# vsois/hanabi-agents

Measured on AMD Instinct MI355X. Metric: env_steps_per_sec, higher is better.
Workload: dtype u8 env/encoder + bfloat16 Q-net GEMM (fp32 accumulate, fp32 master weights)

## Files before the change

### hanabi-agents_amd/csrc/learner2.hip

```cpp
#include <hip/hip_runtime.h>
#include <hip/hip_bf16.h>
#include <hip/hip_fp16.h>

#include <cstdint>
#include <type_traits>

#include "../../include/hanabi_hip.h"
#include "adam_rule.hpp"
#include "common.hpp"

using hb::fail;

namespace {

template <typename T> __device__ __forceinline__ float ld(const T* p, long long i);
template <> __device__ __forceinline__ float ld<float>(const float* p, long long i) { return p[i]; }
template <> __device__ __forceinline__ float ld<__hip_bfloat16>(const __hip_bfloat16* p, long long i) { return __bfloat162float(p[i]); }
template <> __device__ __forceinline__ float ld<__half>(const __half* p, long long i) { return __half2float(p[i]); }
template <typename T> __device__ __forceinline__ void st(T* p, long long i, float v);
template <> __device__ __forceinline__ void st<float>(float* p, long long i, float v) { p[i] = v; }
template <> __device__ __forceinline__ void st<__hip_bfloat16>(__hip_bfloat16* p, long long i, float v) { p[i] = __float2bfloat16(v); }
template <> __device__ __forceinline__ void st<__half>(__half* p, long long i, float v) { p[i] = __float2half(v); }

template <typename T> __device__ __forceinline__ float rounded(float v);
// ... 503 lines not shown
  else return __bfloat162float(b[i]);
}
template <bool F16>
__device__ __forceinline__ tg_f32x4 tg_mfma(const uint4& wv, const uint4& xv, const tg_f32x4& c) {
  if constexpr (F16) {
    union { uint4 u; tg_f16x8 f; } w, x;
    w.u = wv; x.u = xv;
    return __builtin_amdgcn_mfma_f32_16x16x32_f16(w.f, x.f, c, 0, 0, 0);
  } else {
    union { uint4 u; tg_bf16x8 f; } w, x;
    w.u = wv; x.u = xv;
    return __builtin_amdgcn_mfma_f32_16x16x32_bf16(w.f, x.f, c, 0, 0, 0);
  }
}
template <bool F16>
__global__ __launch_bounds__(64) void thin_gemm_kernel(const ThinArgs a, const int batch) {
  const int lane = threadIdx.x;
  const unsigned lr = lane & 15, kq = lane >> 4;
  const unsigned ct = blockIdx.y + a.n_tiles;
  const unsigned c = ct * 16u + 4u * kq;
  const unsigned half = 32u * a.ldx;
#pragma unroll 1
  for (int z = 0; z < batch; ++z) {
    float b0 = 0.f, b1 = 0.f, b2 = 0.f, b3 = 0.f;
    if (a.bias) {
      const __hip_bfloat16* bz = a.bias + static_cast<size_t>(z) * a.nb;
      b0 = tg_bias<F16>(bz, c); b1 = tg_bias<F16>(bz, c + 1); b2 = tg_bias<F16>(bz, c + 2); b3 = tg_bias<F16>(bz, c + 3);
    }
    const unsigned xo = (z * a.x_bs + (blockIdx.x * 32u + lr) * a.ldx + kq * 8u) * 2u;
    const unsigned wo = (z * a.w_bs + (ct * 16u + lr) * a.ldw + kq * 8u) * 2u;
// ... 21 lines not shown
      *reinterpret_cast<uint2*>(o) = make_uint2(tg_pack<F16>(v[0], v[1]), tg_pack<F16>(v[2], v[3]));
      *reinterpret_cast<uint2*>(o + 16u * static_cast<size_t>(a.ldo)) = make_uint2(tg_pack<F16>(v[4], v[5]), tg_pack<F16>(v[6], v[7]));
    }
  }
}

struct TailArgs {
  hb::adam::AdamMulti adam;
  const unsigned char* x;
  const unsigned char* dh;
  unsigned char* dw1;
  int batch, k_rows, hidden;
  unsigned ldx, dh_ld, dw1_ld;
  int g_adam;
  int col_tiles;
};
constexpr int kTailLd = 264;

__device__ __forceinline__ void tail_scatter(uint16_t* lds, int col, int b, const uint4& v) {
  const uint32_t w[4] = {v.x, v.y, v.z, v.w};
#pragma unroll
  for (int i = 0; i < 4; ++i) {
    lds[(col + 2 * i) * kTailLd + b] = static_cast<uint16_t>(w[i] & 0xFFFFu);
    lds[(col + 2 * i + 1) * kTailLd + b] = static_cast<uint16_t>(w[i] >> 16);
  }
}

template <bool F16, int W>
__global__ __launch_bounds__(256) void learner_tail_l2_dw1_kernel(const TailArgs a) {
  typedef typename std::conditional<F16, __half, __hip_bfloat16>::type T;
// ... 1 lines not shown
  __shared__ __attribute__((aligned(16))) uint16_t dt[64 * kTailLd];
  const int tid = static_cast<int>(threadIdx.x);
  if (static_cast<int>(blockIdx.x) < a.g_adam) {
    hb::adam::step_block<T, W>(a.adam, static_cast<int>(blockIdx.x), tid);
    return;
  }
  const int tile = static_cast<int>(blockIdx.x) - a.g_adam;
  const int rt = tile / a.col_tiles, ctile = tile - rt * a.col_tiles;
  const int r0 = rt * 32, c0 = ctile * 64;
  const int kb = (a.batch + 31) & ~31;
  uint4 xv[4], dv[8];
#pragma unroll
  for (int it = 0; it < 4; ++it) {
    const int c = tid + it * 256, b = c >> 2, col = r0 + (c & 3) * 8;
    xv[it] = make_uint4(0u, 0u, 0u, 0u);
    if (b < a.batch && col < a.k_rows) xv[it] = *reinterpret_cast<const uint4*>(a.x + (static_cast<size_t>(b) * a.ldx + col) * 2u);
  }
#pragma unroll
  for (int it = 0; it < 8; ++it) {
    const int c = tid + it * 256, b = c >> 3, col = c0 + (c & 7) * 8;
    dv[it] = make_uint4(0u, 0u, 0u, 0u);
    if (b < a.batch && col < a.hidden) dv[it] = *reinterpret_cast<const uint4*>(a.dh + (static_cast<size_t>(b) * a.dh_ld + col) * 2u);
  }
#pragma unroll
  for (int it = 0; it < 4; ++it) {
    const int c = tid + it * 256, b = c >> 2;
    if (b < kb) tail_scatter(xt, (c & 3) * 8, b, xv[it]);
  }
#pragma unroll
  for (int it = 0; it < 8; ++it) {
    const int c = tid + it * 256, b = c >> 3;
// ... 134 lines not shown
      acc0 = tg_mfma<F16>(w0, x0, acc0);
      acc1 = tg_mfma<F16>(w0, x1, acc1);
      acc0 = tg_mfma<F16>(u0, y0, acc0);
      acc1 = tg_mfma<F16>(u0, y1, acc1);
    }
    if (kb < kend) {
      const uint4 x0 = *reinterpret_cast<const uint4*>(a.x + (xo0 + kb)), x1 = *reinterpret_cast<const uint4*>(a.x + (xo1 + kb));
      const uint4 w0 = *reinterpret_cast<const uint4*>(a.wt + (wo0 + kb));
      acc0 = tg_mfma<F16>(w0, x0, acc0);
      acc1 = tg_mfma<F16>(w0, x1, acc1);
    }
    const size_t ob = z * static_cast<size_t>(a.o_bs) + 4u * kq;
    const size_t o0 = ob + static_cast<size_t>(r0) * a.ldo, o1 = ob + static_cast<size_t>(r1) * a.ldo;
    const __hip_bfloat16* bz = a.bias ? a.bias + static_cast<size_t>(z) * a.nb + 4u * kq : nullptr;
    tf_store<F16>(a.out, a.relu, bz, t0 * 16u, o0, o1, v0, v1, acc0, acc1);
  }
}

}

extern "C" {

int hb_c51_loss_sparse(const void* logits_online_dev, const void* logits_target_dev, int32_t dtype, const int32_t* act_dev,
                       const float* rew_dev, const float* term_dev, const double* prios_dev, const float* beta_dev,
                       const float* disc_dev, int32_t mask_terminal, const float* support_dev, int64_t batch, int32_t n_actions,
                       int32_t n_atoms, int32_t row_stride, float* td_dev, float* w_dev, float* dl_dev, float* update_counter_dev,
                       const void* bias_online_dev, const void* bias_target_dev, void* stream) {
  if (!logits_online_dev || !logits_target_dev || !act_dev || !rew_dev || !term_dev || !prios_dev || !beta_dev || !disc_dev ||
      !support_dev || !td_dev || !w_dev || !dl_dev)
    return fail(HB_ERR_INVALID, "null argument");
// ... 45 lines not shown
  }
  HB_HIP(hipGetLastError());
  return HB_OK;
}

int hb_thin_forward(int32_t layer, const void* x_dev, const void* wt_dev, const void* bias_dev, void* out_dev, const int32_t* act_dev,
                    int64_t batch, int32_t n, int32_t k, int32_t ldx, int32_t ldw, int32_t ldo, int64_t x_batch_stride,
                    int64_t w_batch_stride, int64_t out_batch_stride, int32_t n_actions, int32_t n_atoms, int32_t relu, void* stream) {
  if (!x_dev || !wt_dev || !out_dev) return fail(HB_ERR_INVALID, "null argument");
  if (layer != 1 && layer != 2) return fail(HB_ERR_INVALID, "layer must be 1 or 2");
  if (batch <= 0 || n <= 0) return HB_OK;
  const int64_t m = 2 * batch;
  const int nz = layer == 2 ? 2 : 1;
  if (batch % 32 || n % (layer == 1 ? 32 : 16) || k % 32 || k < 32)
    return fail(HB_ERR_INVALID, "need batch % 32 == 0, n % 16 == 0 (layer 1: n % 32 == 0), k % 32 == 0");
  if (ldx < k || ldw < k || ldo < n || ldx % 8 || ldw % 8 || ldo % 4) return fail(HB_ERR_INVALID, "bad leading dimensions");
  if (relu < 0 || relu > 7) return fail(HB_ERR_INVALID, "relu: bit 0 = ReLU, bit 1 = fp32 output, bit 2 = fp16 (not bf16) operands");
  if ((reinterpret_cast<uintptr_t>(x_dev) & 15u) || (reinterpret_cast<uintptr_t>(wt_dev) & 15u) ||
      (reinterpret_cast<uintptr_t>(out_dev) & ((relu & 2) ? 15u : 7u)))
    return fail(HB_ERR_ALIGN, "x / wt must be 16-byte aligned, out 8-byte (fp32 output: 16-byte) aligned");
  if (layer == 2) {
    if (!act_dev) return fail(HB_ERR_INVALID, "null argument");
    if (batch > 256) return fail(HB_ERR_INVALID, "batch must be <= 256 (a wavefront keeps the batch's actions in four registers per lane)");
    if (n_actions < 1 || n_actions > 64 || n_atoms < 1 || n_atoms > 64 || n_actions * n_atoms > n)
      return fail(HB_ERR_INVALID, "need n_actions <= 64, n_atoms <= 64, n_actions * n_atoms <= n");
    if (x_batch_stride < 0 || w_batch_stride < 0 || out_batch_stride < 0) return fail(HB_ERR_INVALID, "negative batch stride");
    if (x_batch_stride % 8 || w_batch_stride % 8 || out_batch_stride % 4) return fail(HB_ERR_INVALID, "batch strides must keep the alignment");
  }
  const int64_t xe = (nz - 1) * x_batch_stride + m * static_cast<int64_t>(ldx), we = (nz - 1) * w_batch_stride + n * static_cast<int64_t>(ldw);
  if (xe >= (1LL << 30) || we >= (1LL << 30)) return fail(HB_ERR_INVALID, "operands beyond the kernel's 32-bit offsets");
  FwdArgs a{};
  a.x = static_cast<const unsigned char*>(x_dev);
  a.wt = static_cast<const unsigned char*>(wt_dev);
  a.bias = static_cast<const __hip_bfloat16*>(bias_dev);
  a.out = out_dev;
// ... 11 lines not shown
    a.reg0_units = a.nrt * (ncp / 2u);
    a.n_units = a.reg0_units + a.nrt * ncp;
  } else {
    a.x_bs = static_cast<unsigned>(x_batch_stride); a.w_bs = static_cast<unsigned>(w_batch_stride); a.o_bs = static_cast<unsigned>(out_batch_stride);
    a.A = n_actions; a.K = n_atoms;
    a.npair = static_cast<unsigned>((n_atoms + 14) / 16 + 1);
    const unsigned groups = a.nrt + static_cast<unsigned>(n_actions < batch ? n_actions : batch);
    a.n_gather = groups * a.npair;
    a.z[0] = 0u; a.z[1] = 1u;
    a.row0[0] = a.row0[1] = static_cast<unsigned>(batch);
    a.reg0_units = a.nrt * ncp;
    a.n_units = a.n_gather + 2u * a.reg0_units;
  }
  const unsigned per = (a.n_units + 1023u) / 1024u;
  a.stride = (a.n_units + per - 1u) / per;
  if (relu & 4) hipLaunchKernelGGL((thin_forward_kernel<true>), dim3(a.stride), dim3(64), 0, static_cast<hipStream_t>(stream), a);
  else hipLaunchKernelGGL((thin_forward_kernel<false>), dim3(a.stride), dim3(64), 0, static_cast<hipStream_t>(stream), a);
  HB_HIP(hipGetLastError());
  return HB_OK;
}

int hb_dqn_loss_sparse(const void* q_online_dev, const void* q_target_dev, int32_t dtype, const int32_t* act_dev, const float* rew_dev,
                       const float* term_dev, const double* prios_dev, const float* beta_dev, const float* disc_dev, int64_t batch,
                       int32_t n_actions, int32_t col_stride, int32_t row_stride, float* td_dev, float* w_dev, float* dl_dev,
                       const void* bias_online_dev, const void* bias_target_dev, void* stream) {
  if (!q_online_dev || !q_target_dev || !act_dev || !rew_dev || !term_dev || !prios_dev || !beta_dev || !disc_dev || !td_dev ||
      !w_dev || !dl_dev)
    return fail(HB_ERR_INVALID, "null argument");
  if (batch <= 0) return HB_OK;
  if (batch > 256) return fail(HB_ERR_INVALID, "batch must be <= 256");
  if (n_actions < 1 || col_stride < 1 || row_stride < (n_actions - 1) * col_stride + 1) return fail(HB_ERR_INVALID, "bad action layout");
// ... 40 lines not shown

}

int hb::adam::launch_tail(const hb_adam_tensor* steps, int n_steps, const hb_adam_tensor& prod, const float* step_dev,
                          float step_offset, int eff_dtype, float lr, float beta1, float beta2, float eps, void* stream) {
  const int dtype = prod.grad_dtype;
  if (!prod.gdh || !prod.grad) return fail(HB_ERR_INVALID, "gradient product: null gdh / grad");
  if (dtype != 1 && dtype != 2) return fail(HB_ERR_INVALID, "gradient product: grad_dtype must be 1 (bf16) or 2 (f16)");
  if (eff_dtype != dtype) return fail(HB_ERR_INVALID, "gradient product: eff_dtype must equal the product's grad_dtype");
  if (prod.g_batch < 1 || prod.g_batch > 256)
    return fail(HB_ERR_INVALID, "gradient product: g_batch must be 1..256 (a workgroup keeps the tile's operand columns of the whole batch in LDS)");
  if (prod.cols < 8 || prod.cols % 8 || prod.n < prod.cols || prod.n % prod.cols || prod.n / prod.cols >= (1LL << 24))
    return fail(HB_ERR_INVALID, "gradient product: need cols a positive multiple of 8 and n a multiple of cols");
  const int hidden = prod.cols, k_rows = static_cast<int>(prod.n / prod.cols);
  const int ldx = prod.g_ldx, dh_ld = prod.g_ldh, dw1_ld = prod.grad_ld ? prod.grad_ld : prod.cols;
  if (ldx < k_rows || ldx % 8 || dh_ld < hidden || dh_ld % 8 || dw1_ld < hidden || dw1_ld % 4)
    return fail(HB_ERR_INVALID, "gradient product: bad leading dimensions (g_ldx >= n / cols, g_ldh, grad_ld >= cols; g_ldx % 8 == 0, g_ldh % 8 == 0, grad_ld % 4 == 0)");
  if ((reinterpret_cast<uintptr_t>(prod.gx) & 15u) || (reinterpret_cast<uintptr_t>(prod.gdh) & 15u) || (reinterpret_cast<uintptr_t>(prod.grad) & 7u))
    return fail(HB_ERR_ALIGN, "gradient product: gx / gdh must be 16-byte aligned, grad 8-byte aligned");
  TailArgs a{};
  int g_adam = 0, width = 4;
  if (n_steps > 0) {
    width = hb::adam::plan_multi(steps, n_steps, step_dev, step_offset, lr, beta1, beta2, eps, 4, a.adam, &g_adam);
    if (width < 0) return width;
  }
  a.x = static_cast<const unsigned char*>(prod.gx);
  a.dh = static_cast<const unsigned char*>(prod.gdh);
  a.dw1 = static_cast<unsigned char*>(const_cast<void*>(prod.grad));
  a.batch = prod.g_batch; a.k_rows = k_rows; a.hidden = hidden;
  a.ldx = static_cast<unsigned>(ldx); a.dh_ld = static_cast<unsigned>(dh_ld); a.dw1_ld = static_cast<unsigned>(dw1_ld);
  a.g_adam = g_adam;
  a.col_tiles = (hidden + 63) / 64;
  const long long tiles = static_cast<long long>((k_rows + 31) / 32) * a.col_tiles;
  if (tiles + g_adam >= (1LL << 31)) return fail(HB_ERR_INVALID, "too many workgroups");
  const dim3 grid(static_cast<unsigned>(tiles + g_adam)), block(256);
  hipStream_t s = static_cast<hipStream_t>(stream);
  if (dtype == 2 && width == 4) hipLaunchKernelGGL((learner_tail_l2_dw1_kernel<true, 4>), grid, block, 0, s, a);
  else if (dtype == 2) hipLaunchKernelGGL((learner_tail_l2_dw1_kernel<true, 1>), grid, block, 0, s, a);
  else if (width == 4) hipLaunchKernelGGL((learner_tail_l2_dw1_kernel<false, 4>), grid, block, 0, s, a);
  else hipLaunchKernelGGL((learner_tail_l2_dw1_kernel<false, 1>), grid, block, 0, s, a);
  HB_HIP(hipGetLastError());
  return HB_OK;
}
```

### hanabi-agents_amd/csrc/sum_tree.hip

```cpp
#include <hip/hip_runtime.h>
#include <hip/hip_bf16.h>
#include <hip/hip_fp16.h>

#include <cstdlib>
#include <new>

#include "../../include/hanabi_hip.h"
#include "common.hpp"
#include "env_kernel.hpp"

using hb::fail;

struct hb_tree {
  long long cap;
  int depth;
  int chunk;
  float* nodes;
  unsigned* stamp;
  unsigned long long* errors;
  float* scratch;
  long long scratch_n;
  bool single_wg;
  bool fused_pow;
  float* small_scratch;
// ... 378 lines not shown
          j = (j + a.n_ins) % a.ring_cap;
          R += g * a.ring_rew[j];
          g *= a.gamma;
          ++m;
        }
      }
      a.rew[i] = R;
      a.term[i] = a.ring_term[j] ? 1.f : 0.f;
      a.disc[i] = g;
      a.act[i] = a.ring_act[k];
      s_slot[0] = k;
      s_slot[1] = j;
    }
  }
  __syncthreads();
  T* x = static_cast<T*>(a.x);
#pragma unroll
  for (int half = 0; half < 2; ++half) {
    const long long slot = s_slot[half];
    T* dst = x + (static_cast<long long>(half) * B + i) * a.x_ld;
    if (a.packed_words > 0) {
      const uint32_t* src = static_cast<const uint32_t*>(half == 0 ? a.ring_tm1 : a.ring_t) + slot * a.packed_words;
      for (int jj = threadIdx.x; jj < a.L; jj += 256) sg_store<T>(dst, jj, static_cast<float>((src[jj >> 5] >> (jj & 31)) & 1u));
    } else {
      const int8_t* src = static_cast<const int8_t*>(half == 0 ? a.ring_tm1 : a.ring_t) + slot * a.L;
      for (int jj = threadIdx.x; jj < a.L; jj += 256) sg_store<T>(dst, jj, static_cast<float>(src[jj]));
    }
  }
}

__global__ void get_kernel(const float* __restrict__ nodes, long long cap, const int64_t* __restrict__ idx,
                           float* __restrict__ val, long long n, unsigned long long* errors) {
  const long long i = static_cast<long long>(blockIdx.x) * blockDim.x + threadIdx.x;
  if (i >= n) return;
  const long long k = idx[i];
  if (k < 0 || k >= cap) {
    atomicAdd(errors, 1ull);
    val[i] = 0.f;
  } else {
    val[i] = nodes[cap + k];
  }
}
// ... 191 lines not shown
  HB_HIP(hipGetLastError());
  return HB_OK;
}

int hb_per_sample_gather(hb_tree* t, uint64_t seed, const float* counter_dev, int64_t batch, int64_t* idx_dev, double* prob_dev,
                         const void* ring_obs_tm1_dev, const void* ring_obs_t_dev, const int8_t* ring_act_dev,
                         const float* ring_rew_dev, const uint8_t* ring_term_dev, int32_t obs_len, int32_t packed, void* x_dev,
                         int32_t x_dtype, int32_t x_ld, int32_t* act_dev, float* rew_dev, float* term_dev, float* disc_dev,
                         int32_t n_step, float gamma, int64_t capacity, int64_t rows_per_insert, const int64_t* size_wp_dev,
                         void* stream) {
  if (!t) return fail(HB_ERR_INVALID, "null tree");
  if (batch <= 0) return HB_OK;
  if (!counter_dev || !idx_dev || !prob_dev || !ring_obs_tm1_dev || !ring_obs_t_dev || !ring_act_dev || !ring_rew_dev ||
      !ring_term_dev || !x_dev || !act_dev || !rew_dev || !term_dev || !disc_dev)
    return fail(HB_ERR_INVALID, "null argument");
  if (obs_len < 1 || x_ld < obs_len) return fail(HB_ERR_INVALID, "x_ld must be >= obs_len >= 1");
  if (n_step < 1) return fail(HB_ERR_INVALID, "n_step must be >= 1");
  if (n_step > 1 && (!size_wp_dev || rows_per_insert < 1 || capacity < 1))
    return fail(HB_ERR_INVALID, "n_step > 1 needs size_wp_dev, rows_per_insert and capacity");
  SampleGatherArgs a{t->nodes, t->cap, t->depth, static_cast<unsigned long long>(seed), counter_dev, static_cast<int>(batch),
                     idx_dev, prob_dev, ring_obs_tm1_dev, ring_obs_t_dev, ring_act_dev, ring_rew_dev, ring_term_dev, obs_len,
                     packed ? (obs_len + 31) / 32 : 0, x_dev, x_dtype, x_ld, act_dev, rew_dev, term_dev, disc_dev,
                     reinterpret_cast<const long long*>(size_wp_dev), capacity, rows_per_insert, n_step, gamma, 0};
  const int ntop = static_cast<int>(t->cap / t->chunk);
  if (t->lazy_top && ntop > 1) a.ntop = ntop;
  const size_t lds = static_cast<size_t>(2 * a.ntop) * sizeof(float);
  hipStream_t s = static_cast<hipStream_t>(stream);
  const dim3 grid(static_cast<unsigned>(batch)), block(256);
  if (x_dtype == 0) hipLaunchKernelGGL((per_sample_gather_kernel<float>), grid, block, lds, s, a);
  else if (x_dtype == 1) hipLaunchKernelGGL((per_sample_gather_kernel<__hip_bfloat16>), grid, block, lds, s, a);
  else if (x_dtype == 2) hipLaunchKernelGGL((per_sample_gather_kernel<__half>), grid, block, lds, s, a);
  else return fail(HB_ERR_INVALID, "x_dtype must be 0 (f32), 1 (bf16) or 2 (f16)");
  HB_HIP(hipGetLastError());
  return HB_OK;
}

int hb_tree_get(hb_tree* t, const int64_t* idx_dev, float* val_dev, int64_t n, void* stream) {
  if (!t) return fail(HB_ERR_INVALID, "null tree");
  if (n <= 0) return HB_OK;
  if (!idx_dev || !val_dev) return fail(HB_ERR_INVALID, "null argument");
  hipLaunchKernelGGL(get_kernel, dim3(static_cast<unsigned>((n + 255) / 256)), dim3(256), 0,
                     static_cast<hipStream_t>(stream), t->nodes, t->cap, idx_dev, val_dev, static_cast<long long>(n),
                     t->errors);
  HB_HIP(hipGetLastError());
  return HB_OK;
}

// ... 39 lines not shown
```

### hanabi-agents_amd/hanabi_agents/rlax_dqn/fused_learner.py

```python
import os

import torch

from hanabi_hip import _capi as K

_DT = {torch.float32: 0, torch.bfloat16: 1, torch.float16: 2}


class FusedLearner:
    def __init__(self, agent):
        self.agent = agent
        p = agent.params
        dev = agent.device
        self.cd = {"float32": torch.float32, "bfloat16": torch.bfloat16, "float16": torch.float16}[p.compute_dtype]
        self.B = p.train_batch_size
        self.A, self.Kk = agent.atoms.shape
        self.L = agent.obs_len
        layers = agent.online.layers
        assert len(layers) == 2, "the fused learner covers the reference topology: one hidden layer (params.layers=[H])"
        self.layers = layers
        B, AK = self.B, self.A * self.Kk
        H = layers[0].out_features
        f32 = dict(dtype=torch.float32, device=dev)
        pad = (lambda v, m: (v + m - 1) // m * m) if self.cd != torch.float32 else (lambda v, m: v)
# ... 23 lines not shown
        for s in sizes:
            offs.append(offs[-1] + s)
        self.g_w1 = self.flat_grad[offs[0]:offs[1]].view_as(layers[0].w)
        self.g_b1 = self.flat_grad[offs[1]:offs[2]]
        self.g_w2 = self.flat_grad[offs[2]:offs[3]].view_as(layers[1].w)
        self.g_b2 = self.flat_grad[offs[3]:offs[4]]
        self.state = {}
        for li, l in enumerate(layers):
            for name in ("w", "w_mu", "w_sigma", "b", "b_mu", "b_sigma"):
                t = getattr(l, name)
                self.state[(li, name)] = (torch.zeros_like(t), torch.zeros_like(t))
        for li in range(len(layers)):
            self.state[(li, "w_mu")] = self.state[(li, "w")]
            self.state[(li, "b_mu")] = self.state[(li, "b")]
        self.step = torch.zeros((), **f32)
        self.x = torch.zeros(2 * B, self.Kp, dtype=self.cd, device=dev)
        self.act = torch.empty(B, dtype=torch.int32, device=dev)
        self.rew = torch.empty(B, **f32)
        self.term = torch.empty(B, **f32)
        self.disc = torch.empty(B, **f32)
        self.td = torch.empty(B, **f32)
        self.w_is = torch.empty(B, **f32)
        self.dlogits = torch.zeros(B, self.Np, dtype=self.cd, device=dev)
        self.dl = torch.zeros(B, 64, **f32)
        self.dh = torch.zeros(B, H, dtype=self.cd, device=dev)
        self.sparse_backward = self.Kk <= 64 and self.A <= 64 and B <= 256
        self.AK = AK
        self.support = agent.atoms[0].contiguous()
        self._gb2_pad = torch.zeros(self.Np, **f32)
        self._adam_tab = None
        self._idx = self._prob = None
# ... 81 lines not shown
        self.pack_actor()
        if not self.lag:
            return 0
        s = self.n_packed % 2
        if self.packed_ev[s] is not None:
            self.packed_ev[s].wait()
        return s

    @torch.no_grad()
    def refresh_target(self):
        for (w_t, b_t), l in zip(self.trg, self.agent.target.layers):
            self._store(w_t, b_t, *l.effective())
        if self.thin:
            self._transpose(1)

    def sample_and_gather(self, seed):
        a = self.agent
        buf, B = a.experience, self.B
        rpi = buf.rows_per_insert
        c = self._sg_call
        if c is not None and c[0] == (rpi, buf._obs_t_buf.data_ptr()) and c[1] == seed:
            K.check(c[2](*c[3], K.current_stream()))
            return self._idx, self._prob
        L = K.lib()
        if a.params.n_step > 1 and (rpi is None or rpi < 1):
            raise ValueError("n_step > 1 needs inserts of a constant row count (lock-step self-play)")
        if self._idx is None:
            self._idx = torch.empty(B, dtype=torch.int64, device=a.device)
            self._prob = torch.empty(B, dtype=torch.float64, device=a.device)
        args = (buf.sum_tree.h, int(seed), K.dptr(self.step), B, K.dptr(self._idx), K.dptr(self._prob),
                K.dptr(buf._obs_tm1_buf), K.dptr(buf._obs_t_buf), K.dptr(buf._act_tm1_buf),
                K.dptr(buf._rew_t_buf), K.dptr(buf._terminal_t_buf), self.L, 1 if buf.packed else 0,
                K.dptr(self.x), _DT[self.cd], self.Kp, K.dptr(self.act), K.dptr(self.rew), K.dptr(self.term),
                K.dptr(self.disc), int(a.params.n_step), float(a.params.discount), buf.capacity,
                int(rpi or 1), K.dptr(buf._size_wp))
        self._sg_call = ((rpi, buf._obs_t_buf.data_ptr()), seed, L.hb_per_sample_gather, args)
        K.check(L.hb_per_sample_gather(*args, K.current_stream()))
        return self._idx, self._prob

    def _tail_launch(self, adam):
        if self._adam_tab_l2 is None:
            tab = self._adam_table()
            tail, prod = (K.HbAdamTensor * 3)(), (K.HbAdamTensor * 1)()
            tail[0], tail[1], tail[2] = tab[0], tab[2], tab[3]
            prod[0] = tab[0]
            for d in (tail[0], prod[0]):
                d.gx, d.gdh, d.g_batch, d.g_ldx, d.g_ldh = self.x.data_ptr(), self.dh.data_ptr(), self.B, self.Kp, self.H
            self._adam_tab_l2 = (tail, prod)
        p = self.agent.params
        tab, n = (self._adam_tab_l2[0], 3) if adam else (self._adam_tab_l2[1], 1)
        K.check(K.lib().hb_noisy_adam_multi(tab, n, K.dptr(self.step), 0.0, _DT[self.cd], float(p.learning_rate), 0.9, 0.999,
                                            3.125e-5, K.current_stream()))

    def part1(self, indices, prios, gathered=False, defer_dw1=False):
        a, L = self.agent, K.lib()
        buf, B = a.experience, self.B
        if self.direct is None:
            self.direct = not a._collective()
        if self.adam_pack is None:
            self.adam_pack = bool(self.direct and self.thin and not self.lag and self.actor is not None and self.actor.fused
                                  and self.H == 512 and os.environ.get("HB_ADAM_PACK", "0") == "1")
        if self.tail_overlap is None:
            want = os.environ.get("HB_TAIL_OVERLAP", "1" if a.params.n_step == 1 and not self.lag else "0")
            self.tail_overlap = bool(self.direct and self.sparse_backward and not self.adam_pack and self.H % 8 == 0
                                     and self.cd in (torch.bfloat16, torch.float16) and want != "0")
        if a.params.n_step > 1 and (buf.rows_per_insert is None or buf.rows_per_insert < 1):
            raise ValueError("n_step > 1 needs inserts of a constant row count (lock-step self-play)")
        s = K.current_stream()
        if not gathered:
            gather = L.hb_replay_gather_packed if buf.packed else L.hb_replay_gather
            K.check(gather(K.dptr(buf._obs_tm1_buf), K.dptr(buf._obs_t_buf), K.dptr(buf._act_tm1_buf),
                           K.dptr(buf._rew_t_buf), K.dptr(buf._terminal_t_buf), K.dptr(indices), B, self.L,
                           K.dptr(self.x), _DT[self.cd], self.Kp, K.dptr(self.act), K.dptr(self.rew),
                           K.dptr(self.term), K.dptr(self.disc), int(a.params.n_step), float(a.params.discount),
                           buf.capacity, int(buf.rows_per_insert or 1), K.dptr(buf._size_wp), s))
        H = self.H
        w2 = self.eff[1][0]
        if self.thin:
            hcat, logits = self._hcat, self._logits
            if not (self.adam_pack or self.pack_thin):
                self._transpose(0)
            f16 = 4 if self.cd == torch.float16 else 0
            if self.trimmed and self.sparse_backward and not self._dense_forward:
                K.check(L.hb_thin_forward(1, K.dptr(self.x), K.dptr(self.w1catT), K.dptr(self.b1cat), K.dptr(hcat), None, B, 2 * H,
                                          self.Kp, self.Kp, self.Kp, 2 * H, 0, 0, 0, 0, 0, 1 | f16, s))
                K.check(L.hb_thin_forward(2, K.dptr(hcat), K.dptr(self.w2stT), K.dptr(self.b2st), K.dptr(logits), K.dptr(self.act), B,
                                          self.Np, H, 2 * H, H, self.Np, H, self.Np * H, 2 * B * self.Np, self.A, self.Kk, 2 | f16, s))
            else:
                K.check(L.hb_thin_gemm(K.dptr(self.x), K.dptr(self.w1catT), K.dptr(self.b1cat), K.dptr(hcat), 2 * B, 2 * H, self.Kp,
                                       self.Kp, self.Kp, 2 * H, 1, 0, 0, 0, 1 | f16, s))
                K.check(L.hb_thin_gemm(K.dptr(hcat), K.dptr(self.w2stT), K.dptr(self.b2st), K.dptr(logits), 2 * B, self.Np, H, 2 * H, H,
                                       self.Np, 2, H, self.Np * H, 2 * B * self.Np, 2 | f16, s))
        else:
            hcat = torch._addmm_activation(self.b1cat, self.x, self.w1cat, use_gelu=False)
            logits = torch.bmm(hcat.view(2 * B, 2, H).transpose(0, 1), self.w2st)
        logits_on, logits_t = logits[0], logits[1, B:]
        hb, xb = hcat[:B, :H], self.x[:B]
        ldt = 0 if self.thin else _DT[self.cd]
        bon, btg = (None, None) if self.thin else (self.b2st[0], self.b2st[1])
        if self.sparse_backward:
            K.check(L.hb_c51_loss_sparse(K.dptr(logits_on), K.dptr(logits_t), ldt, K.dptr(self.act), K.dptr(self.rew),
                                         K.dptr(self.term), K.dptr(prios), K.dptr(a._beta), K.dptr(self.disc),
                                         1 if a.params.mask_terminal else 0, K.dptr(self.support), B, self.A, self.Kk, self.Np,
                                         K.dptr(self.td), K.dptr(self.w_is), K.dptr(self.dl), K.dptr(self.step),
                                         K.dptr(bon), K.dptr(btg), s))
            K.check(L.hb_c51_backward(K.dptr(self.dl), K.dptr(self.act), K.dptr(hb), hb.stride(0), K.dptr(w2), w2.stride(0),
                                      _DT[self.cd], B, H, self.A, self.Kk, K.dptr(self.dh), K.dptr(self.g_b1),
                                      K.dptr(self._gw2_out), self.Np, K.dptr(self._gb2_pad), s))
            dh = self.dh
        else:
            if self.thin:
                logits_on, logits_t, ldt = logits_on.to(self.cd), logits_t.to(self.cd), _DT[self.cd]
            K.check(L.hb_c51_loss_grad(K.dptr(logits_on), K.dptr(logits_t), ldt, K.dptr(self.act), K.dptr(self.rew),
                                       K.dptr(self.term), K.dptr(prios), K.dptr(a._beta), K.dptr(self.disc),
                                       1 if a.params.mask_terminal else 0, K.dptr(self.support), B, self.A, self.Kk, self.Np,
                                       K.dptr(self.td), K.dptr(self.w_is), K.dptr(self.dlogits), K.dptr(self.step),
                                       K.dptr(bon), K.dptr(btg), s))
            dl = self.dlogits
            torch.mm(hb.t(), dl, out=self._gw2_out)
            K.check(L.hb_colsum(K.dptr(dl), _DT[self.cd], B, self.Np, K.dptr(self._gb2_pad), s))
            dh = torch.mm(dl, w2.t())
            K.check(L.hb_relu_bwd_colsum(K.dptr(dh), K.dptr(hb), hb.stride(0), _DT[self.cd], B, dh.shape[1], K.dptr(self.g_b1), s))
        if self.tail_overlap:
            assert not self._dw1_pending, "part1(defer_dw1=True) must be followed by part2(opt=True) before the next part1"
            self._dw1_pending = bool(defer_dw1)
            if not defer_dw1:
                self._tail_launch(adam=False)
        else:
            torch.mm(xb.t(), dh, out=self._gw1_out)
        if not self.direct:
            self.g_w2.copy_(self._gw2_out[:, :self.AK])
            self.g_b2.copy_(self._gb2_pad[:self.AK])
            self.g_w1.copy_(self._gw1_out[:self.L])
        return self.td, self.w_is

    def _adam_table(self):
        if self._adam_tab is None:
            if self.direct:
                grads = (((self._gw1_out, _DT[self.cd], self._gw1_out.shape[1]), (self.g_b1, 0, 0)),
                         ((self._gw2_out, _DT[self.cd], self.Np), (self._gb2_pad, 0, 0)))
            else:
                grads = (((self.g_w1, 0, 0), (self.g_b1, 0, 0)), ((self.g_w2, 0, 0), (self.g_b2, 0, 0)))
            tab = (K.HbAdamTensor * 4)()
            k = 0
# ... 62 lines not shown
```

### hanabi-agents_amd/hanabi_hip/selfplay.py

```python
import os

import torch

from . import _capi as K

MAX_LEARNER_STREAMS = 2


class SelfPlaySession:
    def __init__(self, env, agents, updates_per_step=1, min_replay=None, train_seats=None, overlap_allreduce=None,
                 learner_stream=True, learner_priority=-1, stream_per_agent=None, fuse_select=True, split_update=True,
                 native_chain=True, early_update=True):
        assert len(agents) == env.players, "one agent per seat"
        self.train_seats = set(range(env.players)) if train_seats is None else set(train_seats)
        self.pool = check_pool_seats(agents, self.train_seats)
        if self.pool is not None:
            self.pool.bind(env, [s for s, a in enumerate(agents) if a is self.pool])
        self._check_color_shuffle(env, agents)
        self.env = env
        self.agents = list(agents)
        self.updates_per_step = int(updates_per_step)
        self.t = 0
        self.last_actions = [torch.zeros(env.n, dtype=torch.int32, device=env.device) for _ in agents]
        self._act_buf = [torch.zeros(env.n, dtype=torch.int32, device=env.device) for _ in agents]
# ... 489 lines not shown
        self.fused_step = session.fuse_env_step and early and env.net_obs.data_ptr() == env.obs_bits.data_ptr()
        act_ptrs = [env.net_obs.data_ptr(), env.legal.data_ptr(), f[0], f[1], f[2], f[3], agent._support0.data_ptr(), act.q.data_ptr(),
                    session._act_buf[seat].data_ptr()]
        if self.fused_step:
            put(K.CMD_ACTOR_FUSED_ACT, A,
                act_ptrs + [env.h, env.reward.data_ptr(), env.terminal.data_ptr(), env.agent_reward.data_ptr(), env.agent_step_type.data_ptr(),
                            env.score.data_ptr()],
                act_ints, var=1, fvar=0)
            put(K.CMD_RECORD_EVENT, A, [acted.h])
        else:
            put(K.CMD_ACTOR_FUSED_ACT, A, act_ptrs, act_ints, var=1, fvar=0)
            put(K.CMD_RECORD_EVENT, A, [acted.h])
            put(K.CMD_ENV_STEP_PACKED, A,
                [env.h, session._act_buf[seat].data_ptr(), env.obs_bits.data_ptr(), None, env.legal.data_ptr(), env.reward.data_ptr(),
                 env.terminal.data_ptr(), env.agent_reward.data_ptr(), env.agent_step_type.data_ptr(), env.score.data_ptr()])
        put(K.CMD_WAIT_EVENT, Ls, [(inserted if early else acted).h])
        put(K.CMD_TREE_FILL_RANGE, Ls, [buf.sum_tree.h, buf._max_priority.data_ptr()], var=2)
        g = fl._sg_call[3]
        put(K.CMD_PER_SAMPLE_GATHER, Ls,
            [g[0], g[2], g[4], g[5], g[6], g[7], g[8], g[9], g[10], g[13], g[16], g[17], g[18], g[19], g[24]],
            [g[1], g[3], g[11], g[12], g[14], g[15], g[20], g[22], g[23]], [g[21]])
        put(K.CMD_RECORD_EVENT, Ls, [agent.gathered_ev.h])
        put(K.CMD_GRAPH_LAUNCH, Ls, [agent._graph1.raw_cuda_graph_exec()])
        if early:
            put(K.CMD_WAIT_EVENT, Ls, [acted.h])
        if agent._graph2 is not None:
            put(K.CMD_GRAPH_LAUNCH, Ls, [agent._graph2.raw_cuda_graph_exec()])
        if self.lag:
            (w1, b1), (w2, b2) = fl.eff
            th = fl._thin_out()
            put(K.CMD_ACTOR_FUSED_PACK, Ls, [w1.data_ptr(), b1.data_ptr(), w2.data_ptr(), b2.data_ptr(), f[0], f[1], f[2], f[3]] +
                ([th[0].data_ptr(), th[2].data_ptr()] if th else [0, 0]),
# ... 17 lines not shown
```

Baseline: 328.7 million.

## Keep sampled learner observations as packed bit rows and expand inside GEMM kernels

```diff
diff --git a/hanabi-agents_amd/csrc/learner2.hip b/hanabi-agents_amd/csrc/learner2.hip
--- a/hanabi-agents_amd/csrc/learner2.hip
+++ b/hanabi-agents_amd/csrc/learner2.hip
@@ -541,6 +541,13 @@
   }
 }
 template <bool F16>
+__device__ __forceinline__ uint4 tg_expand_byte(uint32_t b) {
+  constexpr uint32_t ONE = F16 ? 0x3C00u : 0x3F80u;
+  const uint32_t s = b | (b << 15);
+  return make_uint4(__umul24(s & 0x00010001u, ONE), __umul24(s & 0x00040004u, ONE >> 2), __umul24(s & 0x00100010u, ONE >> 4),
+                    __umul24(s & 0x00400040u, ONE >> 6));
+}
+template <bool F16>
 __global__ __launch_bounds__(64) void thin_gemm_kernel(const ThinArgs a, const int batch) {
   const int lane = threadIdx.x;
   const unsigned lr = lane & 15, kq = lane >> 4;
@@ -592,6 +599,7 @@
   unsigned ldx, dh_ld, dw1_ld;
   int g_adam;
   int col_tiles;
+  int x_bits;
 };
 constexpr int kTailLd = 264;
 
@@ -623,7 +631,10 @@
   for (int it = 0; it < 4; ++it) {
     const int c = tid + it * 256, b = c >> 2, col = r0 + (c & 3) * 8;
     xv[it] = make_uint4(0u, 0u, 0u, 0u);
-    if (b < a.batch && col < a.k_rows) xv[it] = *reinterpret_cast<const uint4*>(a.x + (static_cast<size_t>(b) * a.ldx + col) * 2u);
+    if (b < a.batch && col < a.k_rows) {
+      if (a.x_bits) xv[it] = tg_expand_byte<F16>(a.x[(static_cast<size_t>(b) * a.ldx + rt) * 4u + (c & 3)]);
+      else xv[it] = *reinterpret_cast<const uint4*>(a.x + (static_cast<size_t>(b) * a.ldx + col) * 2u);
+    }
   }
 #pragma unroll
   for (int it = 0; it < 8; ++it) {
@@ -788,6 +799,54 @@
     const size_t o0 = ob + static_cast<size_t>(r0) * a.ldo, o1 = ob + static_cast<size_t>(r1) * a.ldo;
     const __hip_bfloat16* bz = a.bias ? a.bias + static_cast<size_t>(z) * a.nb + 4u * kq : nullptr;
     tf_store<F16>(a.out, a.relu, bz, t0 * 16u, o0, o1, v0, v1, acc0, acc1);
+  }
+}
+
+template <bool F16, int N>
+__device__ __forceinline__ void tfb_round(const unsigned char* xb0, const unsigned char* xb1, const unsigned char* wp, tg_f32x4& acc0,
+                                          tg_f32x4& acc1) {
+  uint32_t b0[N], b1[N];
+  uint4 w[N];
+#pragma unroll
+  for (int t = 0; t < N; ++t) {
+    b0[t] = xb0[4 * t];
+    b1[t] = xb1[4 * t];
+    w[t] = *reinterpret_cast<const uint4*>(wp + 64 * t);
+  }
+  __builtin_amdgcn_sched_barrier(0);
+#pragma unroll
+  for (int t = 0; t < N; ++t) {
+    acc0 = tg_mfma<F16>(w[t], tg_expand_byte<F16>(b0[t]), acc0);
+    acc1 = tg_mfma<F16>(w[t], tg_expand_byte<F16>(b1[t]), acc1);
+  }
+}
+template <bool F16>
+__global__ __launch_bounds__(64) void thin_forward_bits_kernel(const FwdArgs a) {
+#pragma unroll 1
+  for (unsigned u = blockIdx.x; u < a.n_units; u += a.stride) {
+    int lane = threadIdx.x;
+    asm volatile("" : "+v"(lane));
+    const unsigned lr = lane & 15, kq = lane >> 4;
+    unsigned d = u;
+    const unsigned reg = d < a.reg0_units ? 0u : 1u;
+    if (reg) d -= a.reg0_units;
+    const unsigned ct = d / a.nrt, rt = d - ct * a.nrt;
+    const unsigned r0 = a.row0[reg] + 32u * rt + lr, r1 = r0 + 16u;
+    const unsigned xo0 = r0 * a.ldx * 4u + kq, xo1 = r1 * a.ldx * 4u + kq;
+    const unsigned wo0 = ((ct * 16u + lr) * a.ldw + kq * 8u) * 2u;
+    tg_f32x4 acc0 = {0.f, 0.f, 0.f, 0.f}, acc1 = {0.f, 0.f, 0.f, 0.f};
+    const unsigned nk = static_cast<unsigned>(a.k) >> 5;
+    unsigned s = 0;
+#pragma unroll 1
+    for (; s + 4u <= nk; s += 4u) tfb_round<F16, 4>(a.x + (xo0 + 4u * s), a.x + (xo1 + 4u * s), a.wt + (wo0 + 64u * s), acc0, acc1);
+#pragma unroll 1
+    for (; s + 2u <= nk; s += 2u) tfb_round<F16, 2>(a.x + (xo0 + 4u * s), a.x + (xo1 + 4u * s), a.wt + (wo0 + 64u * s), acc0, acc1);
+#pragma unroll 1
+    for (; s < nk; ++s) tfb_round<F16, 1>(a.x + (xo0 + 4u * s), a.x + (xo1 + 4u * s), a.wt + (wo0 + 64u * s), acc0, acc1);
+    const size_t ob = 4u * kq;
+    const size_t o0 = ob + static_cast<size_t>(r0) * a.ldo, o1 = ob + static_cast<size_t>(r1) * a.ldo;
+    const __hip_bfloat16* bz = a.bias ? a.bias + 4u * kq : nullptr;
+    tf_store<F16>(a.out, a.relu, bz, ct * 16u, o0, o1, true, true, acc0, acc1);
   }
 }
 
@@ -863,11 +922,15 @@
   const int nz = layer == 2 ? 2 : 1;
   if (batch % 32 || n % (layer == 1 ? 32 : 16) || k % 32 || k < 32)
     return fail(HB_ERR_INVALID, "need batch % 32 == 0, n % 16 == 0 (layer 1: n % 32 == 0), k % 32 == 0");
-  if (ldx < k || ldw < k || ldo < n || ldx % 8 || ldw % 8 || ldo % 4) return fail(HB_ERR_INVALID, "bad leading dimensions");
+  const bool bits = layer == 1 && n_actions == 1;
+  if (layer == 1 && n_actions != 0 && n_actions != 1) return fail(HB_ERR_INVALID, "layer 1: n_actions must be 0 (16-bit x) or 1 (bit rows)");
+  if (bits) {
+    if (ldx < k / 32 || ldw < k || ldo < n || ldw % 8 || ldo % 4) return fail(HB_ERR_INVALID, "bad leading dimensions (bit rows: ldx in words, ldx >= k / 32)");
+  } else if (ldx < k || ldw < k || ldo < n || ldx % 8 || ldw % 8 || ldo % 4) return fail(HB_ERR_INVALID, "bad leading dimensions");
   if (relu < 0 || relu > 7) return fail(HB_ERR_INVALID, "relu: bit 0 = ReLU, bit 1 = fp32 output, bit 2 = fp16 (not bf16) operands");
-  if ((reinterpret_cast<uintptr_t>(x_dev) & 15u) || (reinterpret_cast<uintptr_t>(wt_dev) & 15u) ||
+  if ((reinterpret_cast<uintptr_t>(x_dev) & (bits ? 3u : 15u)) || (reinterpret_cast<uintptr_t>(wt_dev) & 15u) ||
       (reinterpret_cast<uintptr_t>(out_dev) & ((relu & 2) ? 15u : 7u)))
-    return fail(HB_ERR_ALIGN, "x / wt must be 16-byte aligned, out 8-byte (fp32 output: 16-byte) aligned");
+    return fail(HB_ERR_ALIGN, "x / wt must be 16-byte aligned (bit rows: x 4-byte), out 8-byte (fp32 output: 16-byte) aligned");
   if (layer == 2) {
     if (!act_dev) return fail(HB_ERR_INVALID, "null argument");
     if (batch > 256) return fail(HB_ERR_INVALID, "batch must be <= 256 (a wavefront keeps the batch's actions in four registers per lane)");
@@ -909,7 +972,9 @@
   }
   const unsigned per = (a.n_units + 1023u) / 1024u;
   a.stride = (a.n_units + per - 1u) / per;
-  if (relu & 4) hipLaunchKernelGGL((thin_forward_kernel<true>), dim3(a.stride), dim3(64), 0, static_cast<hipStream_t>(stream), a);
+  if (bits && (relu & 4)) hipLaunchKernelGGL((thin_forward_bits_kernel<true>), dim3(a.stride), dim3(64), 0, static_cast<hipStream_t>(stream), a);
+  else if (bits) hipLaunchKernelGGL((thin_forward_bits_kernel<false>), dim3(a.stride), dim3(64), 0, static_cast<hipStream_t>(stream), a);
+  else if (relu & 4) hipLaunchKernelGGL((thin_forward_kernel<true>), dim3(a.stride), dim3(64), 0, static_cast<hipStream_t>(stream), a);
   else hipLaunchKernelGGL((thin_forward_kernel<false>), dim3(a.stride), dim3(64), 0, static_cast<hipStream_t>(stream), a);
   HB_HIP(hipGetLastError());
   return HB_OK;
@@ -980,10 +1045,14 @@
     return fail(HB_ERR_INVALID, "gradient product: need cols a positive multiple of 8 and n a multiple of cols");
   const int hidden = prod.cols, k_rows = static_cast<int>(prod.n / prod.cols);
   const int ldx = prod.g_ldx, dh_ld = prod.g_ldh, dw1_ld = prod.grad_ld ? prod.grad_ld : prod.cols;
-  if (ldx < k_rows || ldx % 8 || dh_ld < hidden || dh_ld % 8 || dw1_ld < hidden || dw1_ld % 4)
+  if (prod.g_reserved != 0 && prod.g_reserved != 1) return fail(HB_ERR_INVALID, "gradient product: g_reserved must be 0 (16-bit gx) or 1 (bit rows)");
+  const bool bits = prod.g_reserved == 1;
+  if (bits && ldx < (k_rows + 31) / 32)
+    return fail(HB_ERR_INVALID, "gradient product: bad leading dimensions (bit rows: g_ldx in words, g_ldx >= ceil(n / cols / 32))");
+  if ((!bits && (ldx < k_rows || ldx % 8)) || dh_ld < hidden || dh_ld % 8 || dw1_ld < hidden || dw1_ld % 4)
     return fail(HB_ERR_INVALID, "gradient product: bad leading dimensions (g_ldx >= n / cols, g_ldh, grad_ld >= cols; g_ldx % 8 == 0, g_ldh % 8 == 0, grad_ld % 4 == 0)");
-  if ((reinterpret_cast<uintptr_t>(prod.gx) & 15u) || (reinterpret_cast<uintptr_t>(prod.gdh) & 15u) || (reinterpret_cast<uintptr_t>(prod.grad) & 7u))
-    return fail(HB_ERR_ALIGN, "gradient product: gx / gdh must be 16-byte aligned, grad 8-byte aligned");
+  if ((reinterpret_cast<uintptr_t>(prod.gx) & (bits ? 3u : 15u)) || (reinterpret_cast<uintptr_t>(prod.gdh) & 15u) || (reinterpret_cast<uintptr_t>(prod.grad) & 7u))
+    return fail(HB_ERR_ALIGN, "gradient product: gx / gdh must be 16-byte aligned (bit rows: gx 4-byte), grad 8-byte aligned");
   TailArgs a{};
   int g_adam = 0, width = 4;
   if (n_steps > 0) {
@@ -996,6 +1065,7 @@
   a.batch = prod.g_batch; a.k_rows = k_rows; a.hidden = hidden;
   a.ldx = static_cast<unsigned>(ldx); a.dh_ld = static_cast<unsigned>(dh_ld); a.dw1_ld = static_cast<unsigned>(dw1_ld);
   a.g_adam = g_adam;
+  a.x_bits = bits ? 1 : 0;
   a.col_tiles = (hidden + 63) / 64;
   const long long tiles = static_cast<long long>((k_rows + 31) / 32) * a.col_tiles;
   if (tiles + g_adam >= (1LL << 31)) return fail(HB_ERR_INVALID, "too many workgroups");
diff --git a/hanabi-agents_amd/csrc/sum_tree.hip b/hanabi-agents_amd/csrc/sum_tree.hip
--- a/hanabi-agents_amd/csrc/sum_tree.hip
+++ b/hanabi-agents_amd/csrc/sum_tree.hip
@@ -4,6 +4,7 @@
 
 #include <cstdlib>
 #include <new>
+#include <type_traits>
 
 #include "../../include/hanabi_hip.h"
 #include "common.hpp"
@@ -416,6 +417,15 @@
     }
   }
   __syncthreads();
+  if constexpr (std::is_same<T, uint32_t>::value) {
+    uint32_t* x = static_cast<uint32_t*>(a.x);
+    const long long s0 = s_slot[0], s1 = s_slot[1];
+    for (int e = threadIdx.x; e < 2 * a.x_ld; e += 256) {
+      const int half = e >= a.x_ld ? 1 : 0, jj = e - half * a.x_ld;
+      const uint32_t* src = static_cast<const uint32_t*>(half == 0 ? a.ring_tm1 : a.ring_t) + (half == 0 ? s0 : s1) * a.packed_words;
+      x[(static_cast<long long>(half) * B + i) * a.x_ld + jj] = jj < a.packed_words ? src[jj] : 0u;
+    }
+  } else {
   T* x = static_cast<T*>(a.x);
 #pragma unroll
   for (int half = 0; half < 2; ++half) {
@@ -428,6 +438,7 @@
       const int8_t* src = static_cast<const int8_t*>(half == 0 ? a.ring_tm1 : a.ring_t) + slot * a.L;
       for (int jj = threadIdx.x; jj < a.L; jj += 256) sg_store<T>(dst, jj, static_cast<float>(src[jj]));
     }
+  }
   }
 }
 
@@ -649,7 +660,12 @@
   if (!counter_dev || !idx_dev || !prob_dev || !ring_obs_tm1_dev || !ring_obs_t_dev || !ring_act_dev || !ring_rew_dev ||
       !ring_term_dev || !x_dev || !act_dev || !rew_dev || !term_dev || !disc_dev)
     return fail(HB_ERR_INVALID, "null argument");
-  if (obs_len < 1 || x_ld < obs_len) return fail(HB_ERR_INVALID, "x_ld must be >= obs_len >= 1");
+  if (x_dtype < 0 || x_dtype > 3) return fail(HB_ERR_INVALID, "x_dtype must be 0 (f32), 1 (bf16), 2 (f16) or 3 (bit rows)");
+  if (x_dtype == 3) {
+    if (!packed) return fail(HB_ERR_INVALID, "x_dtype 3 (bit rows) needs packed rings");
+    if (obs_len < 1 || x_ld < (obs_len + 31) / 32) return fail(HB_ERR_INVALID, "x_dtype 3: x_ld (words) must be >= ceil(obs_len / 32), obs_len >= 1");
+    if (reinterpret_cast<uintptr_t>(x_dev) & 3u) return fail(HB_ERR_ALIGN, "x_dtype 3: x_dev must be 4-byte aligned");
+  } else if (obs_len < 1 || x_ld < obs_len) return fail(HB_ERR_INVALID, "x_ld must be >= obs_len >= 1");
   if (n_step < 1) return fail(HB_ERR_INVALID, "n_step must be >= 1");
   if (n_step > 1 && (!size_wp_dev || rows_per_insert < 1 || capacity < 1))
     return fail(HB_ERR_INVALID, "n_step > 1 needs size_wp_dev, rows_per_insert and capacity");
@@ -665,7 +681,8 @@
   if (x_dtype == 0) hipLaunchKernelGGL((per_sample_gather_kernel<float>), grid, block, lds, s, a);
   else if (x_dtype == 1) hipLaunchKernelGGL((per_sample_gather_kernel<__hip_bfloat16>), grid, block, lds, s, a);
   else if (x_dtype == 2) hipLaunchKernelGGL((per_sample_gather_kernel<__half>), grid, block, lds, s, a);
-  else return fail(HB_ERR_INVALID, "x_dtype must be 0 (f32), 1 (bf16) or 2 (f16)");
+  else if (x_dtype == 3) hipLaunchKernelGGL((per_sample_gather_kernel<uint32_t>), grid, block, lds, s, a);
+  else return fail(HB_ERR_INVALID, "x_dtype must be 0 (f32), 1 (bf16), 2 (f16) or 3 (bit rows)");
   HB_HIP(hipGetLastError());
   return HB_OK;
 }
diff --git a/hanabi-agents_amd/hanabi_agents/rlax_dqn/fused_learner.py b/hanabi-agents_amd/hanabi_agents/rlax_dqn/fused_learner.py
--- a/hanabi-agents_amd/hanabi_agents/rlax_dqn/fused_learner.py
+++ b/hanabi-agents_amd/hanabi_agents/rlax_dqn/fused_learner.py
@@ -61,7 +61,10 @@
             self.state[(li, "w_mu")] = self.state[(li, "w")]
             self.state[(li, "b_mu")] = self.state[(li, "b")]
         self.step = torch.zeros((), **f32)
-        self.x = torch.zeros(2 * B, self.Kp, dtype=self.cd, device=dev)
+        self._x = None
+        self.bits = None
+        self.xbits = None
+        self._dw1_bits = False
         self.act = torch.empty(B, dtype=torch.int32, device=dev)
         self.rew = torch.empty(B, **f32)
         self.term = torch.empty(B, **f32)
@@ -173,10 +176,38 @@
         if self.thin:
             self._transpose(1)
 
+    @property
+    def x(self):
+        if self._x is None:
+            self._x = torch.zeros(2 * self.B, self.Kp, dtype=self.cd, device=self.agent.device)
+        return self._x
+
+    def _decide(self):
+        if self.bits is not None:
+            return
+        a = self.agent
+        if self.direct is None:
+            self.direct = not a._collective()
+        if self.adam_pack is None:
+            self.adam_pack = bool(self.direct and self.thin and not self.lag and self.actor is not None and self.actor.fused
+                                  and self.H == 512 and os.environ.get("HB_ADAM_PACK", "0") == "1")
+        if self.tail_overlap is None:
+            want = os.environ.get("HB_TAIL_OVERLAP", "1" if a.params.n_step == 1 and not self.lag else "0")
+            self.tail_overlap = bool(self.direct and self.sparse_backward and not self.adam_pack and self.H % 8 == 0
+                                     and self.cd in (torch.bfloat16, torch.float16) and want != "0")
+        want = os.environ.get("HB_LEARNER_BITS", "1" if a.params.n_step == 1 and not self.lag else "0")
+        self.bits = bool(getattr(a.experience, "packed", False) and self.thin and self.trimmed and self.sparse_backward
+                         and self.tail_overlap and not self._dense_forward and want != "0")
+        if self.bits:
+            self.xbits = torch.zeros(2 * self.B, self.Kp // 32, dtype=torch.int32, device=a.device)
+        else:
+            _ = self.x
+
     def sample_and_gather(self, seed):
         a = self.agent
         buf, B = a.experience, self.B
         rpi = buf.rows_per_insert
+        self._decide()
         c = self._sg_call
         if c is not None and c[0] == (rpi, buf._obs_t_buf.data_ptr()) and c[1] == seed:
             K.check(c[2](*c[3], K.current_stream()))
@@ -190,7 +221,8 @@
         args = (buf.sum_tree.h, int(seed), K.dptr(self.step), B, K.dptr(self._idx), K.dptr(self._prob),
                 K.dptr(buf._obs_tm1_buf), K.dptr(buf._obs_t_buf), K.dptr(buf._act_tm1_buf),
                 K.dptr(buf._rew_t_buf), K.dptr(buf._terminal_t_buf), self.L, 1 if buf.packed else 0,
-                K.dptr(self.x), _DT[self.cd], self.Kp, K.dptr(self.act), K.dptr(self.rew), K.dptr(self.term),
+                *((K.dptr(self.xbits), 3, self.Kp // 32) if self.bits else (K.dptr(self.x), _DT[self.cd], self.Kp)),
+                K.dptr(self.act), K.dptr(self.rew), K.dptr(self.term),
                 K.dptr(self.disc), int(a.params.n_step), float(a.params.discount), buf.capacity,
                 int(rpi or 1), K.dptr(buf._size_wp))
         self._sg_call = ((rpi, buf._obs_t_buf.data_ptr()), seed, L.hb_per_sample_gather, args)
@@ -199,30 +231,32 @@
 
     def _tail_launch(self, adam):
         if self._adam_tab_l2 is None:
+            self._adam_tab_l2 = {}
+        bits = self._dw1_bits
+        if bits not in self._adam_tab_l2:
             tab = self._adam_table()
             tail, prod = (K.HbAdamTensor * 3)(), (K.HbAdamTensor * 1)()
             tail[0], tail[1], tail[2] = tab[0], tab[2], tab[3]
             prod[0] = tab[0]
             for d in (tail[0], prod[0]):
-                d.gx, d.gdh, d.g_batch, d.g_ldx, d.g_ldh = self.x.data_ptr(), self.dh.data_ptr(), self.B, self.Kp, self.H
-            self._adam_tab_l2 = (tail, prod)
+                d.gdh, d.g_batch, d.g_ldh = self.dh.data_ptr(), self.B, self.H
+                if bits:
+                    d.gx, d.g_ldx, d.g_reserved = self.xbits.data_ptr(), self.Kp // 32, 1
+                else:
+                    d.gx, d.g_ldx = self.x.data_ptr(), self.Kp
+            self._adam_tab_l2[bits] = (tail, prod)
         p = self.agent.params
-        tab, n = (self._adam_tab_l2[0], 3) if adam else (self._adam_tab_l2[1], 1)
+        tabs = self._adam_tab_l2[bits]
+        tab, n = (tabs[0], 3) if adam else (tabs[1], 1)
         K.check(K.lib().hb_noisy_adam_multi(tab, n, K.dptr(self.step), 0.0, _DT[self.cd], float(p.learning_rate), 0.9, 0.999,
                                             3.125e-5, K.current_stream()))
 
     def part1(self, indices, prios, gathered=False, defer_dw1=False):
         a, L = self.agent, K.lib()
         buf, B = a.experience, self.B
-        if self.direct is None:
-            self.direct = not a._collective()
-        if self.adam_pack is None:
-            self.adam_pack = bool(self.direct and self.thin and not self.lag and self.actor is not None and self.actor.fused
-                                  and self.H == 512 and os.environ.get("HB_ADAM_PACK", "0") == "1")
-        if self.tail_overlap is None:
-            want = os.environ.get("HB_TAIL_OVERLAP", "1" if a.params.n_step == 1 and not self.lag else "0")
-            self.tail_overlap = bool(self.direct and self.sparse_backward and not self.adam_pack and self.H % 8 == 0
-                                     and self.cd in (torch.bfloat16, torch.float16) and want != "0")
+        self._decide()
+        bits = bool(self.bits and gathered)
+        assert not (bits and self._dense_forward), "_dense_forward must be set before the learner's first sample / update"
         if a.params.n_step > 1 and (buf.rows_per_insert is None or buf.rows_per_insert < 1):
             raise ValueError("n_step > 1 needs inserts of a constant row count (lock-step self-play)")
         s = K.current_stream()
@@ -241,8 +275,12 @@
                 self._transpose(0)
             f16 = 4 if self.cd == torch.float16 else 0
             if self.trimmed and self.sparse_backward and not self._dense_forward:
-                K.check(L.hb_thin_forward(1, K.dptr(self.x), K.dptr(self.w1catT), K.dptr(self.b1cat), K.dptr(hcat), None, B, 2 * H,
-                                          self.Kp, self.Kp, self.Kp, 2 * H, 0, 0, 0, 0, 0, 1 | f16, s))
+                if bits:
+                    K.check(L.hb_thin_forward(1, K.dptr(self.xbits), K.dptr(self.w1catT), K.dptr(self.b1cat), K.dptr(hcat), None, B, 2 * H,
+                                              self.Kp, self.Kp // 32, self.Kp, 2 * H, 0, 0, 0, 1, 0, 1 | f16, s))
+                else:
+                    K.check(L.hb_thin_forward(1, K.dptr(self.x), K.dptr(self.w1catT), K.dptr(self.b1cat), K.dptr(hcat), None, B, 2 * H,
+                                              self.Kp, self.Kp, self.Kp, 2 * H, 0, 0, 0, 0, 0, 1 | f16, s))
                 K.check(L.hb_thin_forward(2, K.dptr(hcat), K.dptr(self.w2stT), K.dptr(self.b2st), K.dptr(logits), K.dptr(self.act), B,
                                           self.Np, H, 2 * H, H, self.Np, H, self.Np * H, 2 * B * self.Np, self.A, self.Kk, 2 | f16, s))
             else:
@@ -254,7 +292,7 @@
             hcat = torch._addmm_activation(self.b1cat, self.x, self.w1cat, use_gelu=False)
             logits = torch.bmm(hcat.view(2 * B, 2, H).transpose(0, 1), self.w2st)
         logits_on, logits_t = logits[0], logits[1, B:]
-        hb, xb = hcat[:B, :H], self.x[:B]
+        hb = hcat[:B, :H]
         ldt = 0 if self.thin else _DT[self.cd]
         bon, btg = (None, None) if self.thin else (self.b2st[0], self.b2st[1])
         if self.sparse_backward:
@@ -283,10 +321,11 @@
         if self.tail_overlap:
             assert not self._dw1_pending, "part1(defer_dw1=True) must be followed by part2(opt=True) before the next part1"
             self._dw1_pending = bool(defer_dw1)
+            self._dw1_bits = bits
             if not defer_dw1:
                 self._tail_launch(adam=False)
         else:
-            torch.mm(xb.t(), dh, out=self._gw1_out)
+            torch.mm(self.x[:B].t(), dh, out=self._gw1_out)
         if not self.direct:
             self.g_w2.copy_(self._gw2_out[:, :self.AK])
             self.g_b2.copy_(self._gb2_pad[:self.AK])
diff --git a/hanabi-agents_amd/hanabi_hip/selfplay.py b/hanabi-agents_amd/hanabi_hip/selfplay.py
--- a/hanabi-agents_amd/hanabi_hip/selfplay.py
+++ b/hanabi-agents_amd/hanabi_hip/selfplay.py
@@ -527,8 +527,11 @@
             put(K.CMD_ENV_STEP_PACKED, A,
                 [env.h, session._act_buf[seat].data_ptr(), env.obs_bits.data_ptr(), None, env.legal.data_ptr(), env.reward.data_ptr(),
                  env.terminal.data_ptr(), env.agent_reward.data_ptr(), env.agent_step_type.data_ptr(), env.score.data_ptr()])
+        if early:
+            put(K.CMD_TREE_FILL_RANGE, Ls, [buf.sum_tree.h, buf._max_priority.data_ptr()], var=2)
         put(K.CMD_WAIT_EVENT, Ls, [(inserted if early else acted).h])
-        put(K.CMD_TREE_FILL_RANGE, Ls, [buf.sum_tree.h, buf._max_priority.data_ptr()], var=2)
+        if not early:
+            put(K.CMD_TREE_FILL_RANGE, Ls, [buf.sum_tree.h, buf._max_priority.data_ptr()], var=2)
         g = fl._sg_call[3]
         put(K.CMD_PER_SAMPLE_GATHER, Ls,
             [g[0], g[2], g[4], g[5], g[6], g[7], g[8], g[9], g[10], g[13], g[16], g[17], g[18], g[19], g[24]],
```

Result: slower. 311.0 million (-5.4%).
